# rasd3/TODA

Hardware: AMD Instinct MI355X
Metric: LiDAR training samples/sec (higher is better)
Workload: dtype f32

## Files before the change

toda_amd/csrc/spconv.hip:

```cpp
#include <stdlib.h>

#include <type_traits>

#include <hip/hip_ext.h>

#include <mutex>
#include <vector>

#include "bn_fold.cuh"
#include "common.h"


namespace toda {

typedef float f32x4 __attribute__((ext_vector_type(4)));

constexpr int SC_BLOCK = 256;

static int tiles_pow2(int channels) {
    int t = (channels + 15) / 16, p = 1;
    while (p < t) p <<= 1;
    return p;
}

// ... 538 lines not shown
                    ra[j] = __builtin_bit_cast(f32x4, __builtin_amdgcn_raw_buffer_load_b128(in_rsrc, ok ? (unsigned)qi[ok ? p : d] + (unsigned)(lane % LA) * 16u : OOB, 0, 0));
                }
            }
            if constexpr (STAGE_B) {
#pragma unroll
                for (int j = 0; j < IB; ++j) {
                    const int p = d + lane / LB + (64 / LB) * j;
                    const bool ok = FULL || p < limit;
                    rb[j] = __builtin_bit_cast(f32x4, __builtin_amdgcn_raw_buffer_load_b128(dout_rsrc, ok ? (unsigned)qo[ok ? p : d] + (unsigned)(lane % LB) * 16u : OOB, 0, 0));
                }
            }
#pragma unroll
            for (int t = 0; t < 4; ++t) {
                const int p = d + 4 * t + g;
                const bool ok = FULL || p < limit;
                const int pc = ok ? p : d;
                if constexpr (!STAGE_A) {
#pragma unroll
                    for (int m4 = 0; m4 < MTB; m4 += 4) {
                        const f32x4 v = __builtin_bit_cast(f32x4, __builtin_amdgcn_raw_buffer_load_b128(in_rsrc, ok ? (unsigned)qi[pc] + lane_a + 4u * m4 : OOB, 0, 0));
#pragma unroll
                        for (int m = 0; m < 4; ++m) a[t][m4 + m] = v[m];
                    }
                }
                if constexpr (!STAGE_B) {
#pragma unroll
                    for (int n4 = 0; n4 < NTB; n4 += 4) {
                        const f32x4 v = __builtin_bit_cast(f32x4, __builtin_amdgcn_raw_buffer_load_b128(dout_rsrc, ok ? (unsigned)qo[pc] + lane_b + 4u * n4 : OOB, 0, 0));
#pragma unroll
                        for (int n = 0; n < 4; ++n) b[t][n4 + n] = v[n];
                    }
                }
            }
            if constexpr (STAGE_A) {
#pragma unroll
                for (int j = 0; j < IA; ++j) *reinterpret_cast<f32x4*>(st + (lane / LA + (64 / LA) * j) * (16 * MTB) + (lane % LA) * 4) = ra[j];
            }
            if constexpr (STAGE_B) {
#pragma unroll
                for (int j = 0; j < IB; ++j) *reinterpret_cast<f32x4*>(st + 512 + (lane / LB + (64 / LB) * j) * (16 * NTB) + (lane % LB) * 4) = rb[j];
            }
            __builtin_amdgcn_wave_barrier();
#pragma unroll
            for (int t = 0; t < 4; ++t) {
                if constexpr (STAGE_A) {
#pragma unroll
                    for (int m = 0; m < MTB; ++m) a[t][m] = st[(4 * t + g) * (16 * MTB) + MTB * ii + m];
                }
                if constexpr (STAGE_B) {
#pragma unroll
                    for (int n = 0; n < NTB; ++n) b[t][n] = st[512 + (4 * t + g) * (16 * NTB) + NTB * ii + n];
                }
            }
            __builtin_amdgcn_wave_barrier();
        } else
#pragma unroll
        for (int t = 0; t < 4; ++t) {
            const int p = d + 4 * t + g;
            const bool ok = FULL || p < limit;
            const int pc = ok ? p : d;
            const unsigned ia = (unsigned)qi[pc] + lane_a;
            const unsigned ib = (unsigned)qo[pc] + lane_b;
            if constexpr (EXACT && MTB == 2) {
                const f32x2w v = __builtin_bit_cast(f32x2w, __builtin_amdgcn_raw_buffer_load_b64(in_rsrc, ok ? ia : OOB, 0, 0));
                a[t][0] = v[0], a[t][1] = v[1];
            } else if ((EXACT || exact_a) && MTB % 4 == 0) {
#pragma unroll
                for (int m4 = 0; m4 < MTB; m4 += 4) {
                    const f32x4 v = __builtin_bit_cast(f32x4, __builtin_amdgcn_raw_buffer_load_b128(in_rsrc, ok ? ia + 4u * m4 : OOB, 0, 0));
#pragma unroll
                    for (int m = 0; m < 4; ++m) a[t][m4 + m] = v[m];
                }
            } else {
#pragma unroll
                for (int m = 0; m < MTB; ++m)
                    a[t][m] = __builtin_bit_cast(float, __builtin_amdgcn_raw_buffer_load_b32(
                                  in_rsrc, (ok && (EXACT || MT * ii + m0 + m < cin)) ? ia + 4u * m : OOB, 0, 0));
            }
            if constexpr (EXACT && NTB == 2) {
                const f32x2w v = __builtin_bit_cast(f32x2w, __builtin_amdgcn_raw_buffer_load_b64(dout_rsrc, ok ? ib : OOB, 0, 0));
                b[t][0] = v[0], b[t][1] = v[1];
            } else if ((EXACT || exact_b) && NTB % 4 == 0) {
#pragma unroll
                for (int n4 = 0; n4 < NTB; n4 += 4) {
                    const f32x4 v = __builtin_bit_cast(f32x4, __builtin_amdgcn_raw_buffer_load_b128(dout_rsrc, ok ? ib + 4u * n4 : OOB, 0, 0));
#pragma unroll
                    for (int n = 0; n < 4; ++n) b[t][n4 + n] = v[n];
                }
            } else {
#pragma unroll
                for (int n = 0; n < NTB; ++n)
                    b[t][n] = __builtin_bit_cast(float, __builtin_amdgcn_raw_buffer_load_b32(
                                  dout_rsrc, (ok && (EXACT || NT * ii + n0 + n < cout)) ? ib + 4u * n : OOB, 0, 0));
            }
        }
#pragma unroll
        for (int t = 0; t < 4; ++t) {
            if (FULL || d + 4 * t < limit) {
#pragma unroll
                for (int m = 0; m < MTB; ++m)
#pragma unroll
                    for (int n = 0; n < NTB; ++n)
                        acc[m][n] = __builtin_amdgcn_mfma_f32_16x16x4f32(a[t][m], b[t][n], acc[m][n], 0, 0, 0);
            }
        }
    };

    wg_pair_walk<16>(qi, qo, row_begin + (COOP ? 0 : wv * 64), row_end, COOP ? 64 : SC_BLOCK, nbr + (size_t)k * n_out, n_out, row_a, row_b,
                     lane, std::bool_constant<!COOP>{}, round16);

    for (int src = 1; !COOP && src < SC_BLOCK / 64; ++src) {
        if (wv == src) {
#pragma unroll
            for (int m = 0; m < MTB; ++m)
#pragma unroll
                for (int n = 0; n < NTB; ++n)
#pragma unroll
                    for (int reg = 0; reg < 4; ++reg) red[((m * NTB + n) * 4 + reg) * 64 + lane] = acc[m][n][reg];
        }
        __syncthreads();
        if (wv == 0) {
#pragma unroll
            for (int m = 0; m < MTB; ++m)
#pragma unroll
                for (int n = 0; n < NTB; ++n)
#pragma unroll
                    for (int reg = 0; reg < 4; ++reg) acc[m][n][reg] += red[((m * NTB + n) * 4 + reg) * 64 + lane];
        }
        __syncthreads();
    }
    if (!COOP && wv != 0) return;
    wg_store_slab<true>(acc, slab, chunk, k, K, MT, NT, m0, n0, cin, cout, ii, g);
}

__global__ void __launch_bounds__(SC_BLOCK)
wgrad_reduce_kernel(const float* __restrict__ slab, int chunks, long long elems, float* __restrict__ dw) {
    const long long e = (long long)blockIdx.x * SC_BLOCK + threadIdx.x;
    if (e >= elems) return;
    const float* p = slab + e;
    float s = 0.f;
    int c = 0;
    for (; c + 8 <= chunks; c += 8) {
        float v[8];
#pragma unroll
        for (int i = 0; i < 8; ++i) v[i] = __builtin_nontemporal_load(p + (size_t)(c + i) * elems);
#pragma unroll
        for (int i = 0; i < 8; ++i) s += v[i];
    }
    for (; c < chunks; ++c) s += p[(size_t)c * elems];
    dw[e] = s;
}

#ifndef TODA_CG_WAVES
#define TODA_CG_WAVES 4
#endif
#ifndef TODA_CG_DEPTH
#define TODA_CG_DEPTH 3
#endif
constexpr int CG_WAVES = TODA_CG_WAVES, CG_BLOCK = CG_WAVES * 64, CG_ROWS = CG_BLOCK, CG_K = 27, CG_DEPTH = TODA_CG_DEPTH;

template <int Q, bool VEC>
__global__ void __launch_bounds__(CG_BLOCK)
gather_gemm_compact_kernel(const float* __restrict__ in, int n_in, int cg, const float* __restrict__ w, int w_cout, int w_cin, int transpose,
                           int flip_k, const int* __restrict__ nbr, int n_out, int cp, const float* __restrict__ bias,
                           float* __restrict__ out, double* __restrict__ stats) {
    __shared__ f32x4 w_lds[CG_K * Q * 64];
    __shared__ float acc_lds[CG_WAVES * 65 * 16];
    __shared__ int q_id[CG_WAVES][CG_DEPTH + 1][64];
    __shared__ int q_row[CG_WAVES][CG_DEPTH + 1][64];
    const int tid = threadIdx.x, lane = tid & 63, wv = tid >> 6;
    const int c = lane & 15, g = lane >> 4;
    const int co0 = blockIdx.y * 16;
    const int row0 = blockIdx.x * CG_ROWS + wv * 64;

    const __amdgpu_buffer_rsrc_t id_rsrc = table_rsrc(reinterpret_cast<const float*>(nbr), (unsigned)((size_t)CG_K * n_out * 4u));
    const __amdgpu_buffer_rsrc_t in_rsrc = table_rsrc(in, (unsigned)n_in * (unsigned)cg * 4u);
    int ids[CG_K];
    const bool row_ok = row0 + lane < n_out;
#pragma unroll
    for (int k = 0; k < CG_K; ++k)
        ids[k] = __builtin_bit_cast(int, __builtin_amdgcn_raw_buffer_load_b32(id_rsrc, row_ok ? (unsigned)(((size_t)k * n_out + row0 + lane) * 4u) : OOB, 0, 0));

    {
        constexpr int FR = CG_K * Q * 64, IT = (FR + CG_BLOCK - 1) / CG_BLOCK;
        f32x4 frag[IT];
#pragma unroll
        for (int it = 0; it < IT; ++it) {
            const int e = tid + it * CG_BLOCK;
            const int ln = e & 63, kq = e >> 6;
            const int q = kq % Q, k = kq / Q;
            const int g0 = 16 * q + 4 * (ln >> 4), pch = co0 + (ln & 15);
            const int kk = flip_k ? CG_K - 1 - k : k;
            f32x4 v = f32x4{0.f, 0.f, 0.f, 0.f};
            if (e < FR) {
                if (!transpose) {
                    if (pch < w_cout) {
                        const float* src = w + ((size_t)pch * CG_K + kk) * w_cin + g0;
                        if (VEC && g0 + 3 < w_cin) {
                            v = *reinterpret_cast<const f32x4*>(src);
                        } else {
#pragma unroll
                            for (int j = 0; j < 4; ++j)
                                if (g0 + j < w_cin) v[j] = src[j];
                        }
                    }
                } else if (pch < w_cin) {
#pragma unroll
                    for (int j = 0; j < 4; ++j)
                        if (g0 + j < w_cout) v[j] = w[((size_t)(g0 + j) * CG_K + kk) * w_cin + pch];
                }
            }
            frag[it] = v;
        }
#pragma unroll
        for (int it = 0; it < IT; ++it)
            if (tid + it * CG_BLOCK < FR) w_lds[tid + it * CG_BLOCK] = frag[it];
    }
    {
        const float bv = (bias && co0 + (tid & 15) < cp) ? bias[co0 + (tid & 15)] : 0.f;
        for (int e = tid; e < CG_WAVES * 65 * 16; e += CG_BLOCK) acc_lds[e] = bv;
    }
    __syncthreads();

    struct Stage {
        f32x4 a[Q];
        float s[Q][4];
        int cnt;
    };
    const unsigned long long in_addr = (unsigned long long)in;
    const u32x4 in_desc = {(unsigned)__builtin_amdgcn_readfirstlane((int)(unsigned)in_addr),
                           (unsigned)__builtin_amdgcn_readfirstlane((int)((unsigned)(in_addr >> 32) & 0xFFFFu)),
                           (unsigned)__builtin_amdgcn_readfirstlane((int)((unsigned)n_in * (unsigned)cg * 4u)), 0x00020000u};
    constexpr int LOADS = VEC ? Q : 4 * Q;
    auto prepare = [&](int k, Stage& st) {
        const int i = row_ok ? ids[k] : -1;
        const unsigned long long vote = __ballot(i >= 0);
        int* qi = q_id[wv][k % (CG_DEPTH + 1)];
        int* qr = q_row[wv][k % (CG_DEPTH + 1)];
        st.cnt = __popcll(vote);
        const unsigned long long below = (1ull << lane) - 1;
        const int pos = i >= 0 ? __popcll(vote & below) : st.cnt + __popcll(~vote & below);
        qi[pos] = i;
        qr[pos] = i >= 0 ? lane : 64;
        __builtin_amdgcn_wave_barrier();
        const int src = qi[c];
        const bool ok = src >= 0;
        const unsigned base = (unsigned)src * (unsigned)cg * 4u;
#pragma unroll
        for (int q = 0; q < Q; ++q) {
            if constexpr (VEC) {
                const unsigned off = (ok && 16 * q + 4 * g < cg) ? base + (unsigned)(16 * q + 4 * g) * 4u : OOB;
                asm volatile("buffer_load_dwordx4 %0, %1, %2, 0 offen" : "=v"(st.a[q]) : "v"(off), "s"(in_desc) : "memory");
            } else {
#pragma unroll
                for (int j = 0; j < 4; ++j) {
                    const unsigned off = (ok && 16 * q + 4 * g + j < cg) ? base + (unsigned)(16 * q + 4 * g + j) * 4u : OOB;
                    asm volatile("buffer_load_dword %0, %1, %2, 0 offen" : "=v"(st.s[q][j]) : "v"(off), "s"(in_desc) : "memory");
                }
            }
        }
    };
    auto multiply_add = [&](int k, int tt, int cnt, const f32x4 (&a)[Q]) {
        f32x4 r = f32x4{0.f, 0.f, 0.f, 0.f};
#pragma unroll
        for (int q = 0; q < Q; ++q) {
            const f32x4 b = w_lds[(k * Q + q) * 64 + lane];
#pragma unroll
            for (int j = 0; j < 4; ++j) r = __builtin_amdgcn_mfma_f32_16x16x4f32(a[q][j], b[j], r, 0, 0, 0);
        }
        const i32x4 rows = *reinterpret_cast<const i32x4*>(q_row[wv][k % (CG_DEPTH + 1)] + 16 * tt + 4 * g);
        float* const acc_w = acc_lds + wv * 65 * 16 + c;
        float old[4];
#pragma unroll
        for (int reg = 0; reg < 4; ++reg) old[reg] = acc_w[rows[reg] * 16];
#pragma unroll
        for (int reg = 0; reg < 4; ++reg) acc_w[rows[reg] * 16] = old[reg] + r[reg];
        __builtin_amdgcn_wave_barrier();
    };

    asm volatile("s_waitcnt vmcnt(0)" ::: "memory");
    float dummy = 0.f;
    Stage st[CG_DEPTH];
#pragma unroll
    for (int k = 0; k < CG_DEPTH; ++k) prepare(k, st[k]);
#pragma unroll
    for (int k = 0; k < CG_K; ++k) {
        Stage& ring = st[k % CG_DEPTH];
        if constexpr (VEC) {
            if constexpr (Q == 1)
                asm volatile("s_waitcnt vmcnt(%1)" : "+v"(ring.a[0]) : "n"((CG_DEPTH - 1) * LOADS));
            else
                asm volatile("s_waitcnt vmcnt(%2)" : "+v"(ring.a[0]), "+v"(ring.a[1]) : "n"((CG_DEPTH - 1) * LOADS));
        } else {
#pragma unroll
            for (int q = 0; q < Q; ++q)
                asm volatile("s_waitcnt vmcnt(%4)" : "+v"(ring.s[q][0]), "+v"(ring.s[q][1]), "+v"(ring.s[q][2]), "+v"(ring.s[q][3]) : "n"((CG_DEPTH - 1) * LOADS));
        }
        Stage cur = ring;
        if constexpr (!VEC) {
#pragma unroll
            for (int q = 0; q < Q; ++q) cur.a[q] = f32x4{ring.s[q][0], ring.s[q][1], ring.s[q][2], ring.s[q][3]};
        }
        if (k + CG_DEPTH < CG_K) {
            prepare(k + CG_DEPTH, ring);
        } else {
#pragma unroll
            for (int d = 0; d < LOADS; ++d)
                asm volatile("buffer_load_dword %0, %1, %2, 0 offen" : "+v"(dummy) : "v"(OOB), "s"(in_desc) : "memory");
        }
        multiply_add(k, 0, cur.cnt, cur.a);
        for (int tt = 1; 16 * tt < cur.cnt; ++tt) {
            const int src = q_id[wv][k % (CG_DEPTH + 1)][16 * tt + c];
            const bool ok = src >= 0;
            const unsigned base = (unsigned)src * (unsigned)cg * 4u;
            f32x4 a[Q];
#pragma unroll
            for (int q = 0; q < Q; ++q) {
                if constexpr (VEC) {
                    a[q] = __builtin_bit_cast(f32x4, __builtin_amdgcn_raw_buffer_load_b128(in_rsrc, (ok && 16 * q + 4 * g < cg) ? base + (unsigned)(16 * q + 4 * g) * 4u : OOB, 0, 0));
                } else {
#pragma unroll
                    for (int j = 0; j < 4; ++j)
                        a[q][j] = __builtin_bit_cast(float, __builtin_amdgcn_raw_buffer_load_b32(in_rsrc, (ok && 16 * q + 4 * g + j < cg) ? base + (unsigned)(16 * q + 4 * g + j) * 4u : OOB, 0, 0));
                }
            }
            multiply_add(k, tt, cur.cnt, a);
        }
    }
    asm volatile("s_waitcnt vmcnt(0)" : "+v"(dummy)::"memory");
    __builtin_amdgcn_wave_barrier();
    if (stats) {
        __shared__ float st_sh[2][16][16];
        __syncthreads();
        static_assert(CG_BLOCK % 256 == 0, "one (row group, channel) pair per thread of each 256-thread slice");
        for (int base = 0; base < CG_ROWS; base += 256) {
            float sm = 0.f, sq = 0.f;
            if (tid < 256) {
                const int ch = tid & 15, rg = tid >> 4;
#pragma unroll
                for (int i = 0; i < 16; ++i) {
                    const int R = base + rg * 16 + i;
                    if (blockIdx.x * CG_ROWS + R < n_out) {
                        const float v = acc_lds[((R >> 6) * 65 + (R & 63)) * 16 + ch];
                        sm += v;
                        sq += v * v;
                    }
                }
                st_sh[0][rg][ch] = sm;
                st_sh[1][rg][ch] = sq;
            }
            __syncthreads();
            if (tid < 32) {
                const int qq = tid >> 4, ch = tid & 15;
                double a = 0.0;
#pragma unroll
                for (int rg = 0; rg < 16; ++rg) a += (double)st_sh[qq][rg][ch];
                if (co0 + ch < cp) {
                    double* dst = stats + 2 * cp + (size_t)(qq * cp + co0 + ch) * gridDim.x + blockIdx.x;
                    *dst = base == 0 ? a : *dst + a;
                }
            }
            __syncthreads();
        }
    }
#pragma unroll
    for (int it = 0; it < 4; ++it) {
        const int r = it * 16 + (lane >> 2), c4 = (lane & 3) * 4;
        const f32x4 v = *reinterpret_cast<const f32x4*>(&acc_lds[(wv * 65 + r) * 16 + c4]);
        const int row = row0 + r;
        if (row < n_out) {
            float* dst = out + (size_t)row * cp + co0 + c4;
            if (co0 + c4 + 3 < cp) {
                *reinterpret_cast<f32x4*>(dst) = v;
            } else {
#pragma unroll
                for (int j = 0; j < 4; ++j)
                    if (co0 + c4 + j < cp) dst[j] = v[j];
            }
        }
    }
}

static void wgrad_plan(int n_out, int k_vol, int cin, int cout, int* chunks, int* rows_per_chunk) {
    static const int env_chunks = getenv("TODA_WG_CHUNKS") ? atoi(getenv("TODA_WG_CHUNKS")) : 0;
    int max_chunks = env_chunks > 0 ? env_chunks : ((tiles_pow2(cin) * tiles_pow2(cout) >= 16) ? 48 : 144);
    if (env_chunks <= 0 && k_vol <= 9) max_chunks *= 2;
    int ch = k_vol <= 9 ? n_out / 1024 : n_out / 2048;
    if (ch < 1) ch = 1;
    if (ch > max_chunks) ch = max_chunks;
    if (env_chunks <= 0 && k_vol > 9 && max_chunks == 48 && n_out / 4096 > 48) ch = n_out / 4096 < 96 ? n_out / 4096 : 96;
    if (ch >= 8) ch = (ch + 7) / 8 * 8;
    int rpc = (n_out + ch - 1) / ch;
    rpc = (rpc + 15) / 16 * 16;
    if (rpc < 16) rpc = 16;
    *rows_per_chunk = rpc;
    *chunks = n_out > 0 ? (n_out + rpc - 1) / rpc : 1;
}

}

#include "spconv_split.cuh"

using namespace toda;

#include <atomic>
static std::atomic<int> g_matrix_path{-1};
static int matrix_path() {
    int m = g_matrix_path.load(std::memory_order_relaxed);
    if (m < 0) {
        const char* e = getenv("TODA_MM");
        m = (e && (e[0] == 'n' || e[0] == '0')) ? 0 : 1;
        g_matrix_path.store(m, std::memory_order_relaxed);
    }
    return m;
}
static inline bool use_split(int c_gather, int c_produce) { return matrix_path() == 1 && toda::split_shape_ok(c_gather, c_produce); }

extern "C" int toda_matrix_path(void) { return matrix_path(); }
extern "C" int toda_set_matrix_path(int mode) {
    TODA_CHECK_ARG(mode == 0 || mode == 1, "set_matrix_path: mode must be 0 (native) or 1 (split)");
    g_matrix_path.store(mode, std::memory_order_relaxed);
    return TODA_OK;
}
extern "C" int toda_spconv_split_supported(int c_gather, int c_produce) { return toda::split_shape_ok(c_gather, c_produce) ? 1 : 0; }

extern "C" size_t toda_spconv_packed_weight_floats(int k_vol, int c_gather, int c_produce) {
    const size_t native = (size_t)k_vol * tiles_pow2(c_gather) * tiles_pow2(c_produce) * 256;
    if (!toda::split_shape_ok(c_gather, c_produce)) return native;
    const size_t split = toda::split_packed_bytes(k_vol, c_gather, c_produce) / 4;
    return split > native ? split : native;
}

static void split_pack_fill(toda::SplitPackBatch& b, int i, const float* w, int cout, int k_vol, int cin, int transpose, int flip_k, float* wp) {
    const int cgather = transpose ? cout : cin, cprod = transpose ? cin : cout;
    b.w[i] = w, b.wps[i] = reinterpret_cast<toda::u32x4*>(wp), b.cout[i] = cout, b.K[i] = k_vol, b.cin[i] = cin;
    b.transpose[i] = transpose != 0, b.flip[i] = flip_k != 0;
    b.KC[i] = (unsigned char)(cgather / 32), b.NT[i] = (unsigned char)(cprod / 16);
}

extern "C" int toda_spconv_pack_weight(const float* w, int cout, int k_vol, int cin, int transpose, int flip_k,
                                       float* wp, void* stream) {
    TODA_CHECK_ARG(cout >= 1 && cin >= 1 && k_vol >= 1, "pack_weight: bad shape");
    const int cgather = transpose ? cout : cin, cprod = transpose ? cin : cout;
    TODA_CHECK_ARG(cgather <= 128 && cprod <= 128, "pack_weight: channels > 128 unsupported (gather %d, produce %d)",
                   cgather, cprod);
    if (use_split(cgather, cprod)) {
        toda::SplitPackBatch b = {};
        split_pack_fill(b, 0, w, cout, k_vol, cin, transpose, flip_k, wp);
        hipLaunchKernelGGL(split_pack_batch_kernel, dim3(cdiv((long long)k_vol * b.KC[0] * b.NT[0] * 192, SC_BLOCK), 1), dim3(SC_BLOCK), 0,
                           (hipStream_t)stream, b);
        TODA_LAUNCH_CHECK();
        return TODA_OK;
    }
    const int Q = tiles_pow2(cgather), NT = tiles_pow2(cprod);
    const long long total = (long long)k_vol * Q * NT * 256;
    hipLaunchKernelGGL(pack_weight_kernel, dim3(cdiv(total, SC_BLOCK)), dim3(SC_BLOCK), 0, (hipStream_t)stream, w, cout,
                       k_vol, cin, transpose, flip_k, Q, NT, wp);
    TODA_LAUNCH_CHECK();
    return TODA_OK;
}

extern "C" int toda_spconv_pack_weights(int n, const float* const* w, const int32_t* cout, const int32_t* k_vol, const int32_t* cin,
                                        const int32_t* transpose, const int32_t* flip_k, float* const* wp, void* stream) {
    TODA_CHECK_ARG(n >= 0 && w && cout && k_vol && cin && transpose && flip_k && wp, "pack_weights: null argument");
    PackBatch b = {};
    toda::SplitPackBatch sb = {};
    int m = 0, sm = 0;
    long long most = 0, smost = 0;
    auto flush = [&]() -> int {
        if (m > 0) {
            hipLaunchKernelGGL(pack_weight_batch_kernel, dim3(cdiv(most, SC_BLOCK), m), dim3(SC_BLOCK), 0, (hipStream_t)stream, b);
            TODA_LAUNCH_CHECK();
        }
        m = 0, most = 0;
        return TODA_OK;
    };
    auto sflush = [&]() -> int {
        if (sm > 0) {
            hipLaunchKernelGGL(split_pack_batch_kernel, dim3(cdiv(smost, SC_BLOCK), sm), dim3(SC_BLOCK), 0, (hipStream_t)stream, sb);
            TODA_LAUNCH_CHECK();
        }
        sm = 0, smost = 0;
        return TODA_OK;
    };
    for (int s = 0; s < n; ++s) {
        TODA_CHECK_ARG(w[s] && wp[s] && cout[s] >= 1 && cin[s] >= 1 && k_vol[s] >= 1, "pack_weights: bad segment %d", s);
        const int cgather = transpose[s] ? cout[s] : cin[s], cprod = transpose[s] ? cin[s] : cout[s];
        TODA_CHECK_ARG(cgather <= 128 && cprod <= 128, "pack_weights: channels > 128 unsupported (segment %d)", s);
        if (use_split(cgather, cprod)) {
            split_pack_fill(sb, sm, w[s], cout[s], k_vol[s], cin[s], transpose[s], flip_k[s], wp[s]);
            const long long total = (long long)k_vol[s] * sb.KC[sm] * sb.NT[sm] * 192;
            if (total > smost) smost = total;
            if (++sm == toda::SPLIT_PACK_MAX_SEG) {
                const int rc = sflush();
                if (rc != TODA_OK) return rc;
            }
            continue;
        }
        const int i = m;
        b.w[i] = w[s], b.wp[i] = wp[s], b.cout[i] = cout[s], b.K[i] = k_vol[s], b.cin[i] = cin[s];
        b.transpose[i] = transpose[s] != 0, b.flip[i] = flip_k[s] != 0;
        b.Q[i] = (unsigned char)tiles_pow2(cgather), b.NT[i] = (unsigned char)tiles_pow2(cprod);
        const long long total = (long long)k_vol[s] * b.Q[i] * b.NT[i] * 256;
        if (total > most) most = total;
        if (++m == PACK_MAX_SEG) {
            const int rc = flush();
            if (rc != TODA_OK) return rc;
        }
    }
    {
        const int rc = flush();
        if (rc != TODA_OK) return rc;
    }
    return sflush();
}

namespace toda {
constexpr int CLS_ROWS = 8192, CLS_PER = CLS_ROWS / 256;
struct ClassGeom {
    int stride[3], pad[3];
};
__global__ void __launch_bounds__(256)
class_order_kernel(const int4* __restrict__ coords, int n, const ClassGeom gm, int32_t* __restrict__ order, unsigned char* __restrict__ cls_sorted) {
    __shared__ int cnt[8][256 + 1];
    const int base = blockIdx.x * CLS_ROWS, t = threadIdx.x;
    unsigned char c[CLS_PER];
    int mine[8] = {0, 0, 0, 0, 0, 0, 0, 0};
#pragma unroll
    for (int i = 0; i < CLS_PER; ++i) {
        const int r = base + t * CLS_PER + i;
// ... 177 lines not shown
    return TODA_OK;
}

static int gather_gemm_impl(const float* in, int n_in, int c_gather, const float* wp, const int32_t* nbr, int n_out, int k_vol,
                            int c_produce, const float* bias, float* out, const int32_t* order, double* stats, int* blocks_out, void* stream,
                            const unsigned char* cls_sorted = nullptr, const toda::GatherClasses* cls_table = nullptr) {
    toda::GatherClasses classes = {};
    if (cls_sorted && cls_table) classes = *cls_table;
    else cls_sorted = nullptr;
    TODA_CHECK_ARG(c_gather >= 1 && c_gather <= 128 && c_produce >= 1 && c_produce <= 128,
                   "gather_gemm: channels must be in [1,128] (gather %d, produce %d)", c_gather, c_produce);
    TODA_CHECK_ARG(n_out >= 0 && n_in >= 0 && k_vol >= 1, "gather_gemm: bad sizes");
    TODA_CHECK_ARG((unsigned long long)n_in * c_gather * 4ull < 0xFFFFFFF0ull, "gather_gemm: gathered table must be < 4 GiB");
    if (n_out == 0) return TODA_OK;
    if (n_in == 0) {
        TODA_CHECK_ARG(bias == nullptr, "gather_gemm: empty input with bias is unsupported");
        TODA_HIP(hipMemsetAsync(out, 0, (size_t)n_out * c_produce * sizeof(float), (hipStream_t)stream));
        return TODA_OK;
    }
    GatherRoute r;
    const int rc = gather_route(c_gather, c_produce, n_out, stats != nullptr, cls_sorted != nullptr, &r);
    if (rc != TODA_OK) return rc;
    hipStream_t s = (hipStream_t)stream;
    const dim3 grid(r.grid), block(r.block);
    switch (r.family) {
        case GatherRoute::SPLIT:
            with_tiles(c_gather / 32, c_produce / 16, [&](auto kc, auto nt) {
                constexpr int KC = decltype(kc)::value, NT = decltype(nt)::value;
                if constexpr (KC <= 4 && NT >= 2)
                    GG_LAUNCH(HIP_KERNEL_NAME(gg_split_kernel<KC, NT, (NT == 8 ? 3 : 4), (NT == 2)>), grid, block, 0, s, in, n_in,
                              reinterpret_cast<const toda::u32x4*>(wp), nbr, n_out, k_vol, c_produce, bias, out, order, stats, cls_sorted, classes);
            });
            break;
        case GatherRoute::LDS_128:
            GG_LAUNCH(HIP_KERNEL_NAME(gather_gemm_lds_kernel<8, 8, 1, true, false, 512>), grid, block, 0, s, in, n_in, c_gather, wp, nbr, n_out,
                      k_vol, c_produce, bias, out, order, stats);
            break;
        case GatherRoute::LDS:
            with_tiles(tiles_pow2(c_gather), tiles_pow2(c_produce), [&](auto q, auto nt) {
                constexpr int Q = decltype(q)::value, NT = decltype(nt)::value, RT = NT < 8 ? 2 : 1;
                GG_LAUNCH(HIP_KERNEL_NAME(gather_gemm_lds_kernel<Q, NT, RT, true, true, SC_BLOCK, (Q <= 4 && NT <= 4 && RT == 2)>), grid, block, 0,
                          s, in, n_in, c_gather, wp, nbr, n_out, k_vol, c_produce, bias, out, order, stats);
            });
            break;
        case GatherRoute::REG: {
            auto reg = [&](auto q, auto nt, auto rt, auto vec) {
                constexpr int Q = decltype(q)::value, NT = decltype(nt)::value, RT = decltype(rt)::value;
                constexpr bool VEC = decltype(vec)::value;
                if (cls_sorted && VEC)
                    GG_LAUNCH(HIP_KERNEL_NAME(gather_gemm_kernel<Q, NT, RT, true, true>), grid, block, 0, s, in, n_in, c_gather, wp, nbr, n_out,
                              k_vol, c_produce, bias, out, order, cls_sorted, classes);
                else
                    GG_LAUNCH(HIP_KERNEL_NAME(gather_gemm_kernel<Q, NT, RT, VEC>), grid, block, 0, s, in, n_in, c_gather, wp, nbr, n_out, k_vol,
                              c_produce, bias, out, order, nullptr, classes);
            };
            if (!r.vec) {
                with_tiles(tiles_pow2(c_produce), [&](auto nt) {
                    reg(tile_c<1>{}, nt, tile_c<(decltype(nt)::value < 8 ? 2 : 1)>{}, std::false_type{});
                });
            } else {
                with_tiles(tiles_pow2(c_gather), tiles_pow2(c_produce), [&](auto q, auto nt) {
                    if constexpr (decltype(nt)::value < 8) reg(q, nt, tile_c<2>{}, std::true_type{});
                    else if (r.rt == 2) reg(q, nt, tile_c<2>{}, std::true_type{});
                    else reg(q, nt, tile_c<1>{}, std::true_type{});
                });
            }
            break;
        }
    }
    TODA_LAUNCH_CHECK();
    if (stats) {
        if (blocks_out) {
            *blocks_out = r.grid;
        } else {
            hipLaunchKernelGGL(toda::fold_partials_kernel, dim3(2 * c_produce), dim3(256), 0, s, stats, r.grid, 2 * c_produce);
            TODA_LAUNCH_CHECK();
        }
    }
    return TODA_OK;
}

extern "C" int toda_spconv_gather_gemm_ordered(const float* in, int n_in, int c_gather, const float* wp, const int32_t* nbr,
                                               int n_out, int k_vol, int c_produce, const float* bias, float* out,
                                               const int32_t* order, void* stream) {
    return gather_gemm_impl(in, n_in, c_gather, wp, nbr, n_out, k_vol, c_produce, bias, out, order, nullptr, nullptr, stream);
}

extern "C" int toda_spconv_gather_gemm_classed(const float* in, int n_in, int c_gather, const float* wp, const int32_t* nbr, int n_out, int k_vol,
                                               int c_produce, const float* bias, float* out, const int32_t* order,
                                               const unsigned char* cls_sorted, const int32_t* ksize, const int32_t* stride,
                                               const int32_t* padding, void* stream) {
    TODA_CHECK_ARG(order && cls_sorted && ksize && stride && padding, "gather_gemm_classed: null argument");
    TODA_CHECK_ARG(ksize[0] * ksize[1] * ksize[2] == k_vol, "gather_gemm_classed: kernel size does not match the table's %d offsets", k_vol);
    GatherClasses table;
    TODA_CHECK_ARG(class_table(ksize, stride, padding, &table) == 0, "gather_gemm_classed: needs <= 8 residue classes and <= 27 offsets");
    return gather_gemm_impl(in, n_in, c_gather, wp, nbr, n_out, k_vol, c_produce, bias, out, order, nullptr, nullptr, stream, cls_sorted, &table);
}

extern "C" int toda_spconv_gather_gemm_stats_supported(int c_gather, int c_produce) {
    return gg_stats_supported(c_gather, c_produce) ? 1 : 0;
}

extern "C" size_t toda_spconv_gather_gemm_stats_doubles(int n_out, int c_produce) {
    return (size_t)2 * c_produce * (1 + (size_t)cdiv(n_out > 0 ? n_out : 1, 64));
}

extern "C" int toda_spconv_gather_gemm_stats(const float* in, int n_in, int c_gather, const float* wp, const int32_t* nbr,
                                             int n_out, int k_vol, int c_produce, const float* bias, float* out, double* sums,
                                             size_t sums_doubles, void* stream) {
    TODA_CHECK_ARG(sums != nullptr && gg_stats_supported(c_gather, c_produce) && n_out > 0 && n_in > 0,
                   "gather_gemm_stats: unsupported channel pair (%d -> %d) or empty table", c_gather, c_produce);
    TODA_CHECK_ARG(sums_doubles >= toda_spconv_gather_gemm_stats_doubles(n_out, c_produce), "gather_gemm_stats: statistics buffer too small");
    return gather_gemm_impl(in, n_in, c_gather, wp, nbr, n_out, k_vol, c_produce, bias, out, nullptr, sums, nullptr, stream);
}

extern "C" int toda_spconv_gather_gemm_stats_partials(const float* in, int n_in, int c_gather, const float* wp, const int32_t* nbr,
                                                      int n_out, int k_vol, int c_produce, const float* bias, float* out, double* sums,
                                                      size_t sums_doubles, int* blocks_out, void* stream) {
    TODA_CHECK_ARG(sums != nullptr && blocks_out != nullptr && gg_stats_supported(c_gather, c_produce) && n_out > 0 && n_in > 0,
                   "gather_gemm_stats_partials: unsupported channel pair (%d -> %d), empty table or null argument", c_gather, c_produce);
    TODA_CHECK_ARG(sums_doubles >= toda_spconv_gather_gemm_stats_doubles(n_out, c_produce), "gather_gemm_stats_partials: statistics buffer too small");
    *blocks_out = 0;
    const int rc = gather_gemm_impl(in, n_in, c_gather, wp, nbr, n_out, k_vol, c_produce, bias, out, nullptr, sums, blocks_out, stream);
    if (rc == TODA_OK && *blocks_out <= 0) {
        set_error("gather_gemm_stats_partials: the launch took no statistics");
        return TODA_EINVAL;
    }
    return rc;
}

extern "C" int toda_spconv_gather_gemm(const float* in, int n_in, int c_gather, const float* wp, const int32_t* nbr,
                                       int n_out, int k_vol, int c_produce, const float* bias, float* out,
                                       void* stream) {
    return toda_spconv_gather_gemm_ordered(in, n_in, c_gather, wp, nbr, n_out, k_vol, c_produce, bias, out, nullptr, stream);
}

extern "C" int toda_spconv_gather_gemm_compact_supported(int c_gather, int c_produce, int k_vol) {
    return k_vol == CG_K && c_gather >= 1 && c_gather <= 32 && c_produce >= 1 && c_produce <= 32 && c_produce % 4 == 0;
}

static int gather_gemm_compact_impl(const float* in, int n_in, int c_gather, const float* w, int w_cout, int w_cin, int transpose,
                                    int flip_k, const int32_t* nbr, int n_out, int k_vol, int c_produce, const float* bias,
                                    float* out, double* stats, void* stream) {
    TODA_CHECK_ARG(toda_spconv_gather_gemm_compact_supported(c_gather, c_produce, k_vol),
                   "gather_gemm_compact: needs K = 27, <= 32 gathered and <= 32 produced channels (a multiple of 4) (got K %d, %d -> %d)", k_vol, c_gather,
                   c_produce);
    TODA_CHECK_ARG((transpose ? w_cout : w_cin) == c_gather && (transpose ? w_cin : w_cout) == c_produce,
                   "gather_gemm_compact: weight [%d][27][%d] (transpose %d) does not map %d -> %d channels", w_cout, w_cin, transpose, c_gather, c_produce);
    TODA_CHECK_ARG(n_out >= 0 && n_in >= 0, "gather_gemm_compact: bad sizes");
    TODA_CHECK_ARG((unsigned long long)n_in * c_gather * 4ull < 0xFFFFFFF0ull && (unsigned long long)n_out * CG_K * 4ull < 0xFFFFFFF0ull,
                   "gather_gemm_compact: gathered table and neighbour table must be < 4 GiB each");
    if (n_out == 0) return TODA_OK;
    hipStream_t s = (hipStream_t)stream;
    const dim3 grid(cdiv(n_out, CG_ROWS), cdiv(c_produce, 16));
    const bool vec = c_gather % 4 == 0;
#define CG_LAUNCH(QQ, VV)                                                                                                       \
    hipLaunchKernelGGL(HIP_KERNEL_NAME(gather_gemm_compact_kernel<QQ, VV>), grid, dim3(CG_BLOCK), 0, s, in, n_in, c_gather, w, w_cout, w_cin, \
                       transpose, flip_k, nbr, n_out, c_produce, bias, out, stats)
    if (c_gather <= 16) {
        if (vec) CG_LAUNCH(1, true);
        else CG_LAUNCH(1, false);
    } else {
        if (vec) CG_LAUNCH(2, true);
        else CG_LAUNCH(2, false);
    }
#undef CG_LAUNCH
    TODA_LAUNCH_CHECK();
    return TODA_OK;
}

extern "C" int toda_spconv_gather_gemm_compact(const float* in, int n_in, int c_gather, const float* w, int w_cout, int w_cin, int transpose,
                                               int flip_k, const int32_t* nbr, int n_out, int k_vol, int c_produce, const float* bias,
                                               float* out, void* stream) {
    return gather_gemm_compact_impl(in, n_in, c_gather, w, w_cout, w_cin, transpose, flip_k, nbr, n_out, k_vol, c_produce, bias, out, nullptr, stream);
}

extern "C" size_t toda_spconv_gather_gemm_compact_stats_doubles(int n_out, int c_produce) {
    return (size_t)2 * c_produce * (1 + (size_t)cdiv(n_out > 0 ? n_out : 1, CG_ROWS));
}

extern "C" int toda_spconv_gather_gemm_compact_stats(const float* in, int n_in, int c_gather, const float* w, int w_cout, int w_cin,
                                                     int transpose, int flip_k, const int32_t* nbr, int n_out, int k_vol, int c_produce,
                                                     const float* bias, float* out, double* sums, size_t sums_doubles, int* blocks_out,
                                                     void* stream) {
    TODA_CHECK_ARG(sums != nullptr && n_out > 0, "gather_gemm_compact_stats: null statistics buffer or no output rows");
    TODA_CHECK_ARG(sums_doubles >= toda_spconv_gather_gemm_compact_stats_doubles(n_out, c_produce), "gather_gemm_compact_stats: statistics buffer too small");
    const int rc = gather_gemm_compact_impl(in, n_in, c_gather, w, w_cout, w_cin, transpose, flip_k, nbr, n_out, k_vol, c_produce, bias, out, sums, stream);
    if (rc != TODA_OK) return rc;
    const int blocks = cdiv(n_out, CG_ROWS);
    if (blocks_out) {
        *blocks_out = blocks;
        return TODA_OK;
    }
    hipLaunchKernelGGL(toda::fold_partials_kernel, dim3(2 * c_produce), dim3(256), 0, (hipStream_t)stream, sums, blocks, 2 * c_produce);
    TODA_LAUNCH_CHECK();
    return TODA_OK;
}

extern "C" size_t toda_spconv_wgrad_workspace_bytes(int n_out, int k_vol, int cin, int cout) {
    int chunks, rpc;
    wgrad_plan(n_out, k_vol, cin, cout, &chunks, &rpc);
    return align_up((size_t)chunks * k_vol * cin * cout * sizeof(float), 256);
}

extern "C" int toda_spconv_wgrad(const float* in, int n_in, const float* dout, const int32_t* nbr, int n_out, int k_vol,
                                 int cin, int cout, float* dw, void* ws, size_t ws_bytes, void* stream) {
    TODA_CHECK_ARG(cin >= 1 && cin <= 128 && cout >= 1 && cout <= 128, "wgrad: channels must be in [1,128]");
    TODA_CHECK_ARG(n_out >= 0 && n_in >= 0 && k_vol >= 1, "wgrad: bad sizes");
    TODA_CHECK_ARG((unsigned long long)n_in * cin * 4ull < 0xFFFFFFF0ull && (unsigned long long)n_out * cout * 4ull < 0xFFFFFFF0ull,
                   "wgrad: feature tables must be < 4 GiB");
    hipStream_t s = (hipStream_t)stream;
    const long long elems = (long long)cout * k_vol * cin;
    if (n_out == 0 || n_in == 0) {
        TODA_HIP(hipMemsetAsync(dw, 0, elems * sizeof(float), s));
        return TODA_OK;
    }
    int chunks, rpc;
    wgrad_plan(n_out, k_vol, cin, cout, &chunks, &rpc);
    const size_t need = (size_t)chunks * elems * sizeof(float);
    if (ws_bytes < need) {
        set_error("wgrad: workspace %zu < required %zu", ws_bytes, need);
        return TODA_EWORKSPACE;
    }
    const int MT = tiles_pow2(cin), NT = tiles_pow2(cout);
    static const int env_sub = getenv("TODA_WG_SUB") ? atoi(getenv("TODA_WG_SUB")) : 7;
    static const int env_wg_xcd = getenv("TODA_WG_XCD") ? atoi(getenv("TODA_WG_XCD")) : 1;
    const int chunks_launch = env_wg_xcd ? (chunks + 7) / 8 * 8 : chunks;
    const int xcd_chunks = env_wg_xcd ? chunks_launch : -chunks;
    const bool exact = cin == 16 * MT && cout == 16 * NT;
    float* slab = (float*)ws;

    enum { SPLIT, COOP, TILED } family;
    int mtb = MT < 4 ? MT : 4, ntb = NT < 4 ? NT : 4, nsub_n = 1, grid = chunks_launch * k_vol;
    if (matrix_path() == 1 && toda::wgrad_split_shape_ok(cin, cout)) {
        family = SPLIT;
    } else if (MT == 8 && NT == 8 && (env_sub & 4)) {
        family = COOP, nsub_n = 2;
    } else {
        family = TILED;
        if (MT == 8 && (env_sub & 1)) mtb = 8;
        if (NT == 8 && (env_sub & 2)) ntb = 8;
        nsub_n = NT / ntb;
        grid *= (MT / mtb) * nsub_n;
    }
    auto split = [&](auto kernel) {
        hipLaunchKernelGGL(kernel, dim3(grid), dim3(SC_BLOCK), 0, s, in, n_in, dout, nbr, n_out, k_vol, rpc, slab, xcd_chunks);
    };
    auto native = [&](auto kernel) {
        hipLaunchKernelGGL(kernel, dim3(grid), dim3(SC_BLOCK), 0, s, in, n_in, cin, dout, cout, nbr, n_out, k_vol, rpc, MT, NT, nsub_n, slab,
                           xcd_chunks);
    };
    switch (family) {
        case SPLIT:
            if (cin == 128 && cout == 128) split(wgrad_split_kernel<4, 4, 2, 2>);
            else if (cin == 64 && cout == 128) split(wgrad_split_kernel<4, 4, 1, 2>);
            else if (cin == 128 && cout == 64) split(wgrad_split_kernel<4, 4, 2, 1>);
            else if (cin == 32 && cout == 32) split(wgrad_split_kernel<2, 2>);
            else if (cin == 32) split(wgrad_split_kernel<2, 4>);
            else if (cout == 32) split(wgrad_split_kernel<4, 2>);
            else split(wgrad_split_kernel<4, 4>);
            break;
        case COOP:
            if (exact) native(wgrad_kernel<4, 4, true, true>);
            else native(wgrad_kernel<4, 4, true>);
            break;
        case TILED:
            with_tiles(mtb, ntb, [&](auto m, auto n) {
                constexpr int MTB = decltype(m)::value, NTB = decltype(n)::value;
                if (exact) native(wgrad_kernel<MTB, NTB, false, true>);
                else native(wgrad_kernel<MTB, NTB>);
            });
            break;
    }
    hipLaunchKernelGGL(wgrad_reduce_kernel, dim3(cdiv(elems, SC_BLOCK)), dim3(SC_BLOCK), 0, s, slab, chunks, elems, dw);
    TODA_LAUNCH_CHECK();
    return TODA_OK;
}
```

Baseline: 150.2.

## Compute two 16-channel output tiles per block and double waves per block

Adds an NB template parameter so one block computes two 16-wide output-channel tiles when gathering at most 16 channels but producing more than 16. Each gathered input row is then reused for both tiles instead of being gathered again by a second grid column. Waves per block also go from 4 to 8, and the statistics partials move to fixed 256-row slices so the buffer layout stays independent of block size. This costs more LDS and registers per block, which may lower occupancy.

```diff
diff --git a/toda_amd/csrc/spconv.hip b/toda_amd/csrc/spconv.hip
--- a/toda_amd/csrc/spconv.hip
+++ b/toda_amd/csrc/spconv.hip
@@ -714,20 +714,21 @@
 }
 
 #ifndef TODA_CG_WAVES
-#define TODA_CG_WAVES 4
+#define TODA_CG_WAVES 8
 #endif
 #ifndef TODA_CG_DEPTH
 #define TODA_CG_DEPTH 3
 #endif
 constexpr int CG_WAVES = TODA_CG_WAVES, CG_BLOCK = CG_WAVES * 64, CG_ROWS = CG_BLOCK, CG_K = 27, CG_DEPTH = TODA_CG_DEPTH;
-
-template <int Q, bool VEC>
+constexpr int CG_STAT_ROWS = 256;
+
+template <int Q, bool VEC, int NB = 1>
 __global__ void __launch_bounds__(CG_BLOCK)
 gather_gemm_compact_kernel(const float* __restrict__ in, int n_in, int cg, const float* __restrict__ w, int w_cout, int w_cin, int transpose,
                            int flip_k, const int* __restrict__ nbr, int n_out, int cp, const float* __restrict__ bias,
                            float* __restrict__ out, double* __restrict__ stats) {
-    __shared__ f32x4 w_lds[CG_K * Q * 64];
-    __shared__ float acc_lds[CG_WAVES * 65 * 16];
+    __shared__ f32x4 w_lds[NB * CG_K * Q * 64];
+    __shared__ float acc_lds[NB * CG_WAVES * 65 * 16];
     __shared__ int q_id[CG_WAVES][CG_DEPTH + 1][64];
     __shared__ int q_row[CG_WAVES][CG_DEPTH + 1][64];
     const int tid = threadIdx.x, lane = tid & 63, wv = tid >> 6;
@@ -744,14 +745,14 @@
         ids[k] = __builtin_bit_cast(int, __builtin_amdgcn_raw_buffer_load_b32(id_rsrc, row_ok ? (unsigned)(((size_t)k * n_out + row0 + lane) * 4u) : OOB, 0, 0));
 
     {
-        constexpr int FR = CG_K * Q * 64, IT = (FR + CG_BLOCK - 1) / CG_BLOCK;
+        constexpr int FR = NB * CG_K * Q * 64, IT = (FR + CG_BLOCK - 1) / CG_BLOCK;
         f32x4 frag[IT];
 #pragma unroll
         for (int it = 0; it < IT; ++it) {
             const int e = tid + it * CG_BLOCK;
             const int ln = e & 63, kq = e >> 6;
-            const int q = kq % Q, k = kq / Q;
-            const int g0 = 16 * q + 4 * (ln >> 4), pch = co0 + (ln & 15);
+            const int q = kq % Q, k = (kq / Q) % CG_K, nb = kq / (Q * CG_K);
+            const int g0 = 16 * q + 4 * (ln >> 4), pch = co0 + 16 * nb + (ln & 15);
             const int kk = flip_k ? CG_K - 1 - k : k;
             f32x4 v = f32x4{0.f, 0.f, 0.f, 0.f};
             if (e < FR) {
@@ -778,9 +779,10 @@
         for (int it = 0; it < IT; ++it)
             if (tid + it * CG_BLOCK < FR) w_lds[tid + it * CG_BLOCK] = frag[it];
     }
-    {
-        const float bv = (bias && co0 + (tid & 15) < cp) ? bias[co0 + (tid & 15)] : 0.f;
-        for (int e = tid; e < CG_WAVES * 65 * 16; e += CG_BLOCK) acc_lds[e] = bv;
+#pragma unroll
+    for (int nb = 0; nb < NB; ++nb) {
+        const float bv = (bias && co0 + 16 * nb + (tid & 15) < cp) ? bias[co0 + 16 * nb + (tid & 15)] : 0.f;
+        for (int e = tid; e < CG_WAVES * 65 * 16; e += CG_BLOCK) acc_lds[nb * CG_WAVES * 65 * 16 + e] = bv;
     }
     __syncthreads();
 
@@ -823,20 +825,29 @@
         }
     };
     auto multiply_add = [&](int k, int tt, int cnt, const f32x4 (&a)[Q]) {
-        f32x4 r = f32x4{0.f, 0.f, 0.f, 0.f};
+        f32x4 r[NB];
+#pragma unroll
+        for (int nb = 0; nb < NB; ++nb) r[nb] = f32x4{0.f, 0.f, 0.f, 0.f};
 #pragma unroll
         for (int q = 0; q < Q; ++q) {
-            const f32x4 b = w_lds[(k * Q + q) * 64 + lane];
-#pragma unroll
-            for (int j = 0; j < 4; ++j) r = __builtin_amdgcn_mfma_f32_16x16x4f32(a[q][j], b[j], r, 0, 0, 0);
+            f32x4 b[NB];
+#pragma unroll
+            for (int nb = 0; nb < NB; ++nb) b[nb] = w_lds[((nb * CG_K + k) * Q + q) * 64 + lane];
+#pragma unroll
+            for (int j = 0; j < 4; ++j)
+#pragma unroll
+                for (int nb = 0; nb < NB; ++nb) r[nb] = __builtin_amdgcn_mfma_f32_16x16x4f32(a[q][j], b[nb][j], r[nb], 0, 0, 0);
         }
         const i32x4 rows = *reinterpret_cast<const i32x4*>(q_row[wv][k % (CG_DEPTH + 1)] + 16 * tt + 4 * g);
-        float* const acc_w = acc_lds + wv * 65 * 16 + c;
-        float old[4];
-#pragma unroll
-        for (int reg = 0; reg < 4; ++reg) old[reg] = acc_w[rows[reg] * 16];
-#pragma unroll
-        for (int reg = 0; reg < 4; ++reg) acc_w[rows[reg] * 16] = old[reg] + r[reg];
+        float old[NB][4];
+#pragma unroll
+        for (int nb = 0; nb < NB; ++nb)
+#pragma unroll
+            for (int reg = 0; reg < 4; ++reg) old[nb][reg] = acc_lds[(nb * CG_WAVES + wv) * 65 * 16 + c + rows[reg] * 16];
+#pragma unroll
+        for (int nb = 0; nb < NB; ++nb)
+#pragma unroll
+            for (int reg = 0; reg < 4; ++reg) acc_lds[(nb * CG_WAVES + wv) * 65 * 16 + c + rows[reg] * 16] = old[nb][reg] + r[nb][reg];
         __builtin_amdgcn_wave_barrier();
     };
 
@@ -894,50 +905,56 @@
     if (stats) {
         __shared__ float st_sh[2][16][16];
         __syncthreads();
-        static_assert(CG_BLOCK % 256 == 0, "one (row group, channel) pair per thread of each 256-thread slice");
-        for (int base = 0; base < CG_ROWS; base += 256) {
-            float sm = 0.f, sq = 0.f;
-            if (tid < 256) {
-                const int ch = tid & 15, rg = tid >> 4;
-#pragma unroll
-                for (int i = 0; i < 16; ++i) {
-                    const int R = base + rg * 16 + i;
-                    if (blockIdx.x * CG_ROWS + R < n_out) {
-                        const float v = acc_lds[((R >> 6) * 65 + (R & 63)) * 16 + ch];
-                        sm += v;
-                        sq += v * v;
+        static_assert(CG_BLOCK % CG_STAT_ROWS == 0 && CG_STAT_ROWS == 256, "one (row group, channel) pair per thread of each 256-thread slice");
+        const int slices = (n_out + 255) / 256;
+#pragma unroll
+        for (int nb = 0; nb < NB; ++nb) {
+            for (int base = 0; base < CG_ROWS; base += 256) {
+                const int slice = blockIdx.x * (CG_ROWS / 256) + base / 256;
+                if (slice >= slices) break;
+                float sm = 0.f, sq = 0.f;
+                if (tid < 256) {
+                    const int ch = tid & 15, rg = tid >> 4;
+#pragma unroll
+                    for (int i = 0; i < 16; ++i) {
+                        const int R = base + rg * 16 + i;
+                        if (blockIdx.x * CG_ROWS + R < n_out) {
+                            const float v = acc_lds[((nb * CG_WAVES + (R >> 6)) * 65 + (R & 63)) * 16 + ch];
+                            sm += v;
+                            sq += v * v;
+                        }
                     }
-                }
-                st_sh[0][rg][ch] = sm;
-                st_sh[1][rg][ch] = sq;
-            }
-            __syncthreads();
-            if (tid < 32) {
-                const int qq = tid >> 4, ch = tid & 15;
-                double a = 0.0;
-#pragma unroll
-                for (int rg = 0; rg < 16; ++rg) a += (double)st_sh[qq][rg][ch];
-                if (co0 + ch < cp) {
-                    double* dst = stats + 2 * cp + (size_t)(qq * cp + co0 + ch) * gridDim.x + blockIdx.x;
-                    *dst = base == 0 ? a : *dst + a;
-                }
-            }
-            __syncthreads();
-        }
-    }
-#pragma unroll
-    for (int it = 0; it < 4; ++it) {
-        const int r = it * 16 + (lane >> 2), c4 = (lane & 3) * 4;
-        const f32x4 v = *reinterpret_cast<const f32x4*>(&acc_lds[(wv * 65 + r) * 16 + c4]);
-        const int row = row0 + r;
-        if (row < n_out) {
-            float* dst = out + (size_t)row * cp + co0 + c4;
-            if (co0 + c4 + 3 < cp) {
-                *reinterpret_cast<f32x4*>(dst) = v;
-            } else {
-#pragma unroll
-                for (int j = 0; j < 4; ++j)
-                    if (co0 + c4 + j < cp) dst[j] = v[j];
+                    st_sh[0][rg][ch] = sm;
+                    st_sh[1][rg][ch] = sq;
+                }
+                __syncthreads();
+                if (tid < 32) {
+                    const int qq = tid >> 4, ch = tid & 15;
+                    double a = 0.0;
+#pragma unroll
+                    for (int rg = 0; rg < 16; ++rg) a += (double)st_sh[qq][rg][ch];
+                    if (co0 + 16 * nb + ch < cp) stats[2 * cp + (size_t)(qq * cp + co0 + 16 * nb + ch) * slices + slice] = a;
+                }
+                __syncthreads();
+            }
+        }
+    }
+#pragma unroll
+    for (int nb = 0; nb < NB; ++nb) {
+#pragma unroll
+        for (int it = 0; it < 4; ++it) {
+            const int r = it * 16 + (lane >> 2), c4 = 16 * nb + (lane & 3) * 4;
+            const f32x4 v = *reinterpret_cast<const f32x4*>(&acc_lds[((nb * CG_WAVES + wv) * 65 + r) * 16 + (lane & 3) * 4]);
+            const int row = row0 + r;
+            if (row < n_out) {
+                float* dst = out + (size_t)row * cp + co0 + c4;
+                if (co0 + c4 + 3 < cp) {
+                    *reinterpret_cast<f32x4*>(dst) = v;
+                } else {
+#pragma unroll
+                    for (int j = 0; j < 4; ++j)
+                        if (co0 + c4 + j < cp) dst[j] = v[j];
+                }
             }
         }
     }
@@ -1421,17 +1438,21 @@
                    "gather_gemm_compact: gathered table and neighbour table must be < 4 GiB each");
     if (n_out == 0) return TODA_OK;
     hipStream_t s = (hipStream_t)stream;
-    const dim3 grid(cdiv(n_out, CG_ROWS), cdiv(c_produce, 16));
+    const bool both = c_produce > 16 && c_gather <= 16;
+    const dim3 grid(cdiv(n_out, CG_ROWS), both ? 1 : cdiv(c_produce, 16));
     const bool vec = c_gather % 4 == 0;
-#define CG_LAUNCH(QQ, VV)                                                                                                       \
-    hipLaunchKernelGGL(HIP_KERNEL_NAME(gather_gemm_compact_kernel<QQ, VV>), grid, dim3(CG_BLOCK), 0, s, in, n_in, c_gather, w, w_cout, w_cin, \
+#define CG_LAUNCH(QQ, VV, NN)                                                                                                      \
+    hipLaunchKernelGGL(HIP_KERNEL_NAME(gather_gemm_compact_kernel<QQ, VV, NN>), grid, dim3(CG_BLOCK), 0, s, in, n_in, c_gather, w, w_cout, w_cin, \
                        transpose, flip_k, nbr, n_out, c_produce, bias, out, stats)
-    if (c_gather <= 16) {
-        if (vec) CG_LAUNCH(1, true);
-        else CG_LAUNCH(1, false);
+    if (both) {
+        if (vec) CG_LAUNCH(1, true, 2);
+        else CG_LAUNCH(1, false, 2);
+    } else if (c_gather <= 16) {
+        if (vec) CG_LAUNCH(1, true, 1);
+        else CG_LAUNCH(1, false, 1);
     } else {
-        if (vec) CG_LAUNCH(2, true);
-        else CG_LAUNCH(2, false);
+        if (vec) CG_LAUNCH(2, true, 1);
+        else CG_LAUNCH(2, false, 1);
     }
 #undef CG_LAUNCH
     TODA_LAUNCH_CHECK();
@@ -1445,7 +1466,7 @@
 }
 
 extern "C" size_t toda_spconv_gather_gemm_compact_stats_doubles(int n_out, int c_produce) {
-    return (size_t)2 * c_produce * (1 + (size_t)cdiv(n_out > 0 ? n_out : 1, CG_ROWS));
+    return (size_t)2 * c_produce * (1 + (size_t)cdiv(n_out > 0 ? n_out : 1, CG_STAT_ROWS));
 }
 
 extern "C" int toda_spconv_gather_gemm_compact_stats(const float* in, int n_in, int c_gather, const float* w, int w_cout, int w_cin,
@@ -1456,7 +1477,7 @@
     TODA_CHECK_ARG(sums_doubles >= toda_spconv_gather_gemm_compact_stats_doubles(n_out, c_produce), "gather_gemm_compact_stats: statistics buffer too small");
     const int rc = gather_gemm_compact_impl(in, n_in, c_gather, w, w_cout, w_cin, transpose, flip_k, nbr, n_out, k_vol, c_produce, bias, out, sums, stream);
     if (rc != TODA_OK) return rc;
-    const int blocks = cdiv(n_out, CG_ROWS);
+    const int blocks = cdiv(n_out, CG_STAT_ROWS);
     if (blocks_out) {
         *blocks_out = blocks;
         return TODA_OK;
```

Result: no change. 151.3 (median of 6 runs) (+0.7%).
